# taohan10200/CRA5

Measured on AMD Instinct MI355X. Metric: ERA5 frames/s (721x1440x268) encode+decode, higher is better.
Workload: dtype f32 (3xf16-split MFMA, fp32 accumulate)

## Files before the change

cra5_amd/csrc/attention_split_f16.hip:

```cpp
#include <hip/hip_runtime.h>
#include <math.h>
#include <stdlib.h>

#include "../../include/cra5_amd.h"
#include "split.h"

CRA5_RANGE_TU(attn)

typedef float f32x16 __attribute__((ext_vector_type(16)));
typedef _Float16 half8 __attribute__((ext_vector_type(8)));
typedef _Float16 half4 __attribute__((ext_vector_type(4)));
typedef __fp16 fp16x4 __attribute__((__vector_size__(4 * sizeof(__fp16))));
#if defined(__HIP_DEVICE_COMPILE__)
#define CRA5_TR_READ(P) \
  __builtin_bit_cast(half4, __builtin_amdgcn_ds_read_tr16_b64_v4f16((__attribute__((address_space(3))) fp16x4 *)(P)))
#else
#define CRA5_TR_READ(P) (*reinterpret_cast<const half4 *>(P))
#endif

namespace {

__device__ __forceinline__ int xcd_remap(int bid, int nb) {
  const int q = nb / 8, r = nb % 8;
  const int xcd = bid % 8, within = bid / 8;
  const int base = (xcd < r) ? xcd * (q + 1) : r * (q + 1) + (xcd - r) * q;
  return base + within;
}

struct WinGeom {
  int H, W, wh, ww, nwc;
};

__device__ __forceinline__ int token_of(const WinGeom &g, int wr, int wc, int t) {
  if (g.ww == g.W && g.wh == g.H) return t;
  const int r = t / g.ww, c = t - r * g.ww;
  const int gr = wr * g.wh + r, gc = wc * g.ww + c;
  return (gr < g.H && gc < g.W) ? gr * g.W + gc : -1;
}

#ifdef CRA5_ATTN_TRACE
__device__ unsigned long long g_attn_trace[6 * 8192];
#define CRA5_ATRACE(SLOT, VAL)                                                                          \
  if (threadIdx.x == 0 && atrace_idx < 8192) g_attn_trace[atrace_idx * 6 + (SLOT)] = (VAL);
#else
#define CRA5_ATRACE(SLOT, VAL)
#endif

constexpr int HD = 64;
constexpr int KS = 72;
constexpr int VS = 96;
constexpr int MAX_WIN_TOKENS = 1152;

struct BalArgs {
  int groups;
  int n_full;
  int n_wg_pass;
  int rem_tile0;
  int rem;
  int n_grp;
  int nkt;
  int maxp;
  float *ws;
};
__host__ __device__ __forceinline__ long bal_cut(long S, int G, int c) { return S * c / G; }
__host__ __device__ __forceinline__ int bal_piece_of(long S, int G, long s) {
  int c = (int)(s * G / S);
  if (c > G - 1) c = G - 1;
  while (c > 0 && bal_cut(S, G, c) > s) --c;
  while (c < G - 1 && bal_cut(S, G, c + 1) <= s) ++c;
  return c;
}
constexpr int WS_ROW = 68;

template <int NW, bool HI, bool GLOBAL, bool BAL = false, bool PLAIN = false>
__global__ __launch_bounds__(NW * 64, (NW >= 8 ? 1 : (NW == 4 ? 3 : 2))) void window_attention_split_kernel(
    const unsigned short *__restrict__ qkv, long ldq ,
    const unsigned short *__restrict__ pad_row, float *__restrict__ out, unsigned short *__restrict__ out_s,
    int Kp_out, int C, int heads, WinGeom g, int q_tiles , float scale, BalArgs bal) {
  static_assert(!BAL || GLOBAL, "the balanced schedule is for whole-grid launches");
  static_assert(!PLAIN || HI, "plain rows carry no lo plane");
  constexpr int NT = NW * 64;
  constexpr int PPR = PLAIN ? 8 : 16;
  constexpr int PIECES = 32 * PPR;
  constexpr int STG = (PIECES + NT - 1) / NT;

  constexpr int KPL = 32 * KS + 32;
  constexpr int VPL = 32 * VS;
  constexpr int KBUF = 2 * KPL, VBUF = 2 * VPL;
  __shared__ __attribute__((aligned(16))) unsigned short lds[2 * KBUF + 2 * VBUF];
  unsigned short *Ks = lds;
  unsigned short *Vt = lds + 2 * KBUF;
  constexpr int TAB = GLOBAL ? 1 : MAX_WIN_TOKENS;
  __shared__ long long tab[TAB];

  const int L = g.wh * g.ww;
  int head, win, n_seg = 1;
  int seg_tile0[2] = {0, 0}, seg_nact[2] = {NW, NW}, seg_j0[2] = {0, 0}, seg_j1[2] = {L / 32, L / 32}, seg_part[2] = {-1, -1};
  int seg_grp[2] = {0, 0};
  if (BAL) {
    const int pass = blockIdx.x / bal.n_wg_pass, w = blockIdx.x - pass * bal.n_wg_pass;
    int slot;
    if ((heads & 7) == 0 && (bal.n_wg_pass & 7) == 0) {
      const int xcd = w & 7, s_ = w >> 3;
      head = xcd * (heads >> 3) + s_ / bal.groups;
      slot = s_ % bal.groups;
    } else {
      head = w / bal.groups;
      slot = w % bal.groups;
    }
    win = 0;
    if (pass < bal.n_full) {
      seg_tile0[0] = (pass * bal.groups + slot) * NW;
    } else {
      const long S = (long)bal.n_grp * bal.nkt;
      const long s0 = bal_cut(S, bal.groups, slot), s1 = bal_cut(S, bal.groups, slot + 1);
      n_seg = 0;
      for (long s = s0; s < s1;) {
        const int gq = (int)(s / bal.nkt);
        const long e = min(s1, (long)(gq + 1) * bal.nkt);
        if (n_seg < 2) {
          seg_grp[n_seg] = gq;
          seg_tile0[n_seg] = bal.rem_tile0 + gq * NW;
          seg_nact[n_seg] = min(NW, bal.rem - gq * NW);
          seg_j0[n_seg] = (int)(s - (long)gq * bal.nkt);
          seg_j1[n_seg] = (int)(e - (long)gq * bal.nkt);
          seg_part[n_seg] = slot - bal_piece_of(S, bal.groups, (long)gq * bal.nkt);
          ++n_seg;
        }
        s = e;
      }
    }
  } else {
    const int pid = xcd_remap(blockIdx.x, gridDim.x);
    const int qt = pid % q_tiles;
    const int wh_id = pid / q_tiles;
    head = wh_id % heads;
    win = wh_id / heads;
    seg_tile0[0] = qt * NW;
  }
  const int wr = win / g.nwc, wc = win - wr * g.nwc;

  const int tid = threadIdx.x, lane = tid & 63, wave = tid >> 6;
  const int l31 = lane & 31, h = lane >> 5;
  const int hoff = head * HD;
  const long qoff = (PLAIN ? 1L : 2L) * hoff, koff = (PLAIN ? 1L : 2L) * (C + hoff), voff = (PLAIN ? 1L : 2L) * (2 * C + hoff);

  if (!GLOBAL) {
    const long long pad_delta = reinterpret_cast<const char *>(pad_row) - reinterpret_cast<const char *>(qkv);
    for (int t = tid; t < L; t += NT) {
      const int tok = token_of(g, wr, wc, t);
      tab[t] = (tok >= 0) ? (long long)tok * ldq * 2 : pad_delta;
    }
  }
  constexpr bool IDLE_SKIP = !GLOBAL || BAL;
  bool tab_ready = GLOBAL;
#pragma unroll 1
  for (int seg = 0; seg < n_seg; ++seg) {
  const int tile0 = seg_tile0[seg], n_active = seg_nact[seg], j0 = seg_j0[seg], j1 = seg_j1[seg];
#ifdef CRA5_ATTN_TRACE
  const int atrace_idx = GLOBAL ? 8192 : (int)blockIdx.x;
  const unsigned long long atrace_c0 = clock64();
#endif
  CRA5_ATRACE(0, wall_clock64());
  const int tq = (tile0 + wave) * 32 + l31;
  const int q_tok = (tq < L && wave < n_active) ? token_of(g, wr, wc, tq) : -1;
  const bool wave_active = __any(q_tok >= 0);
  if (!__syncthreads_or(wave_active ? 1 : 0)) continue;
  tab_ready = true;

  half8 qh[4], ql[4];
  {
    const unsigned short *qrow = ((q_tok >= 0) ? qkv + (size_t)q_tok * ldq : pad_row) + qoff;
#pragma unroll
    for (int s = 0; s < 4; ++s) {
      const int chunk = s >> 1, pp = 2 * (s & 1) + h;
      if (PLAIN) {
        qh[s] = *reinterpret_cast<const half8 *>(qrow + 16 * s + 8 * h);
        ql[s] = qh[s];
      } else {
        qh[s] = *reinterpret_cast<const half8 *>(qrow + chunk * 64 + pp * 8);
        ql[s] = *reinterpret_cast<const half8 *>(qrow + chunk * 64 + 32 + pp * 8);
      }
    }
  }
  const float cexp = scale * 1.44269504088896340736f;
  f32x16 negm;
#pragma unroll
  for (int r = 0; r < 16; ++r) negm[r] = 0.f;
  if (HI) {
#pragma unroll
    for (int s = 0; s < 4; ++s)
#pragma unroll
      for (int e = 0; e < 8; ++e) qh[s][e] = (_Float16)((float)qh[s][e] * cexp);
  }
  const float cmax = HI ? 1.0f : cexp;

  f32x16 o[2];
#pragma unroll
  for (int t = 0; t < 2; ++t)
#pragma unroll
    for (int r = 0; r < 16; ++r) o[t][r] = 0.f;
  float m_run = HI ? 0.f : -INFINITY, l_run = 0.f;

  const int n_tiles = j1 - j0;
  uint4 sk0 = make_uint4(0u, 0u, 0u, 0u), sk1 = sk0, sv0 = sk0, sv1 = sk0;
  static_assert(STG == 1 || STG == 2, "staging below is written out for one or two 16-byte pieces per thread");
  constexpr bool TWO = STG == 2;
  const int krow0 = min(tid / PPR, 31), krow1 = min((tid + NT) / PPR, 31);
  const long kcol = koff + (tid % PPR) * 8;
  const long vcol = voff + (tid % PPR) * 8;
  const unsigned short *kq0 = qkv + (size_t)(krow0 + 32 * j0) * ldq + kcol;
  const unsigned short *kq1 = qkv + (size_t)(krow1 + 32 * j0) * ldq + kcol;
  const unsigned short *vq0 = qkv + (size_t)(krow0 + 32 * j0) * ldq + vcol;
  const unsigned short *vq1 = qkv + (size_t)(krow1 + 32 * j0) * ldq + vcol;
  const long tile_step = 32 * ldq;
#define CRA5_ROW(JJ, ROW) \
  reinterpret_cast<const unsigned short *>(reinterpret_cast<const char *>(qkv) + tab[(JJ)*32 + (ROW)])
  const bool stage0 = (NT <= PIECES) || (tid < PIECES);
  const bool stage1 = TWO && (tid + NT < PIECES);
#define CRA5_K_LOAD(J)                                                                    \
  if (stage0) {                                                                           \
    if (GLOBAL) {                                                                         \
      sk0 = *reinterpret_cast<const uint4 *>(kq0);                                        \
      if (stage1) sk1 = *reinterpret_cast<const uint4 *>(kq1);                            \
      const long st_ = ((J) < n_tiles - 1) ? tile_step : 0;  \
      kq0 += st_;                                                                         \
      kq1 += st_;                                                                         \
    } else {                                                                              \
      const int jj_ = min((J), n_tiles - 1);                                              \
      sk0 = *reinterpret_cast<const uint4 *>(CRA5_ROW(jj_, krow0) + kcol);                \
      if (stage1) sk1 = *reinterpret_cast<const uint4 *>(CRA5_ROW(jj_, krow1) + kcol);    \
    }                                                                                     \
  }
#define CRA5_V_LOAD(J)                                                                    \
  if (stage0) {                                                                           \
    if (GLOBAL) {                                                                         \
      sv0 = *reinterpret_cast<const uint4 *>(vq0);                                        \
      if (stage1) sv1 = *reinterpret_cast<const uint4 *>(vq1);                            \
      const long st_ = ((J) < n_tiles - 1) ? tile_step : 0;                               \
      vq0 += st_;                                                                         \
      vq1 += st_;                                                                         \
    } else {                                                                              \
      const int jj_ = min((J), n_tiles - 1);                                              \
      sv0 = *reinterpret_cast<const uint4 *>(CRA5_ROW(jj_, krow0) + vcol);                \
      if (stage1) sv1 = *reinterpret_cast<const uint4 *>(CRA5_ROW(jj_, krow1) + vcol);    \
    }                                                                                     \
  }
#define CRA5_K_STORE1(P, BUF)                                                             \
  {                                                                                       \
    const int idx = tid + (P)*NT;                                                         \
    if (idx < PIECES) {                                                                   \
      const int row = idx / PPR, piece = idx % PPR;                                       \
      const int plane = PLAIN ? 0 : (piece >> 2) & 1, d0 = PLAIN ? 8 * piece : 32 * (piece >> 3) + 8 * (piece & 3); \
      *reinterpret_cast<uint4 *>(Ks + (BUF)*KBUF + plane * KPL + row * KS + d0) = sk##P;  \
    }                                                                                     \
  }
#define CRA5_K_STORE(BUF) { CRA5_K_STORE1(0, BUF) if (TWO) CRA5_K_STORE1(1, BUF) }
#define CRA5_V_STORE1(P, BUF)                                                             \
  {                                                                                       \
    const int idx = tid + (P)*NT;                                                         \
    if (idx < PIECES) {                                                                   \
      const int row = idx / PPR, piece = idx % PPR;                                       \
      const int plane = PLAIN ? 0 : (piece >> 2) & 1, d0 = PLAIN ? 8 * piece : 32 * (piece >> 3) + 8 * (piece & 3); \
      *reinterpret_cast<uint4 *>(Vt + (BUF)*VBUF + plane * VPL + row * VS + d0) = sv##P;  \
    }                                                                                     \
  }
#define CRA5_V_STORE(BUF) { CRA5_V_STORE1(0, BUF) if (TWO) CRA5_V_STORE1(1, BUF) }
#define CRA5_SCORES(DST, KB)                                                              \
  {                                                                                       \
    f32x16 acc_;                                                                          \
    _Pragma("unroll") for (int r = 0; r < 16; ++r) acc_[r] = 0.f;                         \
    _Pragma("unroll") for (int st = 0; st < 4; ++st) {                                    \
      const half8 kh = *reinterpret_cast<const half8 *>(k_base + (KB)*KBUF + 16 * st);     \
      const half8 kl = *reinterpret_cast<const half8 *>(k_base + (KB)*KBUF + KPL + 16 * st); \
      if (!HI) {                                                                          \
        acc_ = __builtin_amdgcn_mfma_f32_32x32x16_f16(kl, qh[st], acc_, 0, 0, 0);         \
        acc_ = __builtin_amdgcn_mfma_f32_32x32x16_f16(kh, ql[st], acc_, 0, 0, 0);         \
      }                                                                                   \
      if (HI && st == 0) {                                                                \
        CRA5_MFMA_FROM(acc_, kh, qh[0], negm);                                            \
      } else {                                                                            \
        acc_ = __builtin_amdgcn_mfma_f32_32x32x16_f16(kh, qh[st], acc_, 0, 0, 0);         \
      }                                                                                   \
    }                                                                                     \
    DST = acc_;                                                                           \
  }
#if defined(__HIP_DEVICE_COMPILE__)
#define CRA5_MFMA_FROM(D, A, B, C) \
  asm("s_nop 3\n\tv_mfma_f32_32x32x16_f16 %0, %1, %2, %3" : "=&v"(D) : "v"(A), "v"(B), "v"(C))
#else
#define CRA5_MFMA_FROM(D, A, B, C) (D) = (C)
#endif

  const unsigned short *k_base = Ks + l31 * KS + 8 * h;
  const unsigned short *v_base = Vt + (4 * h + ((lane & 15) >> 2)) * VS + 16 * ((lane >> 4) & 1) + 4 * (lane & 3);

#if defined(__HIP_DEVICE_COMPILE__)
#define CRA5_XHALF_MAX(X)                                                                 \
  ({                                                                                      \
    float a_ = (X), b_ = (X), r_;                                                         \
    asm("s_nop 1\n\tv_permlane32_swap_b32_e32 %0, %1\n\ts_nop 1\n\tv_max_f32_e32 %2, %0, %1" \
        : "+v"(a_), "+v"(b_), "=v"(r_));                                                  \
    r_;                                                                                   \
  })
#define CRA5_MAX2_VALU(A, B)                                                              \
  ({                                                                                      \
    float r_;                                                                             \
    asm("v_max_f32_e32 %0, %1, %2" : "=v"(r_) : "v"(A), "v"(B));                          \
    r_;                                                                                   \
  })
#else
#define CRA5_XHALF_MAX(X) (X)
#define CRA5_MAX2_VALU(A, B) fmaxf((A), (B))
#endif
#if !defined(__HIP_DEVICE_COMPILE__)
#define CRA5_TILE_MAX(S)                                                                  \
  ({                                                                                      \
    float m_ = fmaxf(fmaxf(fmaxf(S[0], S[1]), fmaxf(S[2], S[3])), fmaxf(fmaxf(S[4], S[5]), fmaxf(S[6], S[7]))); \
    float n_ = fmaxf(fmaxf(fmaxf(S[8], S[9]), fmaxf(S[10], S[11])), fmaxf(fmaxf(S[12], S[13]), fmaxf(S[14], S[15]))); \
    CRA5_XHALF_MAX(fmaxf(m_, n_)) * cmax;       \
  })
#else
#define CRA5_MAX3(A, B, C) fmaxf(fmaxf((A), (B)), (C))
#define CRA5_TILE_MAX(S)                                                                  \
  ({                                                                                      \
    const float a_ = CRA5_MAX3(S[0], S[1], S[2]), b_ = CRA5_MAX3(S[3], S[4], S[5]), c_ = CRA5_MAX3(S[6], S[7], S[8]); \
    const float d_ = CRA5_MAX3(S[9], S[10], S[11]), e_ = CRA5_MAX3(S[12], S[13], S[14]);     \
    const float f_ = CRA5_MAX3(a_, b_, c_), g_ = CRA5_MAX3(d_, e_, S[15]);                   \
    CRA5_XHALF_MAX(CRA5_MAX2_VALU(f_, g_)) * cmax;  \
  })
#endif

  f32x16 s_cur;
  CRA5_K_LOAD(0);
  CRA5_V_LOAD(0);
  CRA5_K_STORE(0);
  CRA5_V_STORE(0);
  CRA5_K_LOAD(1);
  CRA5_K_STORE(1);
  __syncthreads();
  CRA5_K_LOAD(2);
  CRA5_V_LOAD(1);
  CRA5_SCORES(s_cur, 0);
  float mloc = CRA5_TILE_MAX(s_cur);
  __syncthreads();

  auto key_tile = [&](const int j, f32x16 &s_cur, f32x16 &s_next) __attribute__((always_inline)) {
    const int kb = (j + 1) & 1, vb = j & 1;
    if (!IDLE_SKIP || wave_active) {
    constexpr float DEFER_LOG2 = 8.0f;
    auto shift = [&](float delta, const bool rescale, f32x16 *also) __attribute__((always_inline)) {
      delta = (float)(_Float16)fminf(fmaxf(delta, -60000.f), 60000.f);
      if (rescale) {
        const float alpha = __builtin_amdgcn_exp2f(-delta);
        l_run *= alpha;
#pragma unroll
        for (int t = 0; t < 2; ++t)
#pragma unroll
          for (int r = 0; r < 16; ++r) o[t][r] *= alpha;
      }
      m_run += delta;
      half8 e0, bd;
#pragma unroll
      for (int e = 0; e < 8; ++e) {
        e0[e] = (_Float16)0.0f;
        bd[e] = (_Float16)0.0f;
      }
      e0[0] = (_Float16)(h == 0 ? 1.0f : 0.0f);
      bd[0] = (_Float16)(h == 0 ? -delta : 0.0f);
      s_cur = __builtin_amdgcn_mfma_f32_32x32x16_f16(e0, bd, s_cur, 0, 0, 0);
      negm = __builtin_amdgcn_mfma_f32_32x32x16_f16(e0, bd, negm, 0, 0, 0);
      if (also) *also = __builtin_amdgcn_mfma_f32_32x32x16_f16(e0, bd, *also, 0, 0, 0);
#if defined(__HIP_DEVICE_COMPILE__)
      asm volatile("s_nop 15\n\ts_nop 3" ::: "memory");
#endif
    };
    if (HI) {
      if (j == 0) shift(mloc, false, nullptr);
    } else if (!__all(mloc - m_run <= DEFER_LOG2)) {
      const float m_new = fmaxf(m_run, mloc);
      const float alpha = __builtin_amdgcn_exp2f(m_run - m_new);
      l_run *= alpha;
#pragma unroll
      for (int t = 0; t < 2; ++t)
#pragma unroll
        for (int r = 0; r < 16; ++r) o[t][r] *= alpha;
      m_run = m_new;
    }
    const float m_new = m_run;
#if defined(__HIP_DEVICE_COMPILE__)
    if (!HI) {
#define CRA5_FENCE() __builtin_amdgcn_sched_barrier(0)
#define CRA5_STAGE(MFMA_STMT) \
  CRA5_FENCE();               \
  MFMA_STMT;                  \
  CRA5_FENCE();
#define CRA5_KFRAG(PLANE, ST) (*reinterpret_cast<const half8 *>(k_base + kb * KBUF + (PLANE)*KPL + 16 * (ST)))
#define CRA5_MM(A, B, C) __builtin_amdgcn_mfma_f32_32x32x16_f16((A), (B), (C), 0, 0, 0)
      typedef _Float16 half2v __attribute__((ext_vector_type(2)));
      typedef unsigned u32x4 __attribute__((ext_vector_type(4)));
      float p[16], psum = 0.f;
      u32x4 phw[2], plw[2];
      auto exp_half = [&](const int u) __attribute__((always_inline)) {
        p[2 * u] = __builtin_amdgcn_exp2f(fmaf(s_cur[2 * u], cexp, -m_new));
        p[2 * u + 1] = __builtin_amdgcn_exp2f(fmaf(s_cur[2 * u + 1], cexp, -m_new));
      };
      auto split_half = [&](const int u) __attribute__((always_inline)) {
        const int r = 2 * u;
        const half2v h2 = {(_Float16)p[r], (_Float16)p[r + 1]};
        const unsigned hh = __builtin_bit_cast(unsigned, h2);
        float d0, d1;
        asm("v_fma_mix_f32 %0, %2, -1.0, %3 op_sel_hi:[1,0,0]\n\t"
            "v_fma_mix_f32 %1, %2, -1.0, %4 op_sel:[1,0,0] op_sel_hi:[1,0,0]"
            : "=&v"(d0), "=&v"(d1) : "v"(hh), "v"(p[r]), "v"(p[r + 1]));
        psum += p[r];
        psum += p[r + 1];
        const half2v l2 = {(_Float16)d0, (_Float16)d1};
        unsigned ll = __builtin_bit_cast(unsigned, l2);
        asm("" : "+v"(ll));
        phw[u >> 2][u & 3] = hh;
        plw[u >> 2][u & 3] = ll;
      };
#define ph(T) __builtin_bit_cast(half8, phw[T])
#define pl(T) __builtin_bit_cast(half8, plw[T])
      half8 vh[2], vl[2];
      auto v_frag = [&](const int t, const int plane, const int dt) __attribute__((always_inline)) {
        const unsigned short *vp = v_base + vb * VBUF + plane * VPL + 16 * t * VS + 32 * dt;
        const half4 a0 = CRA5_TR_READ(vp);
        const half4 a1 = CRA5_TR_READ(vp + 8 * VS);
        return __builtin_shufflevector(a0, a1, 0, 1, 2, 3, 4, 5, 6, 7);
      };
      half8 kh0 = CRA5_KFRAG(0, 0), kl0 = CRA5_KFRAG(1, 0), kh1 = CRA5_KFRAG(0, 1), kl1 = CRA5_KFRAG(1, 1);
      f32x16 acc;
#pragma unroll
      for (int r = 0; r < 16; ++r) acc[r] = 0.f;
      CRA5_STAGE(acc = CRA5_MM(kl0, qh[0], acc))
      exp_half(0);
      CRA5_STAGE(acc = CRA5_MM(kh0, ql[0], acc))
      exp_half(1);
      CRA5_STAGE(acc = CRA5_MM(kh0, qh[0], acc))
      split_half(0);
      const half8 kh2 = CRA5_KFRAG(0, 2), kl2 = CRA5_KFRAG(1, 2);
      CRA5_STAGE(acc = CRA5_MM(kl1, qh[1], acc))
      exp_half(2);
      CRA5_STAGE(acc = CRA5_MM(kh1, ql[1], acc))
      split_half(1);
      CRA5_STAGE(acc = CRA5_MM(kh1, qh[1], acc))
      exp_half(3);
      const half8 kh3 = CRA5_KFRAG(0, 3), kl3 = CRA5_KFRAG(1, 3);
      CRA5_STAGE(acc = CRA5_MM(kl2, qh[2], acc))
      split_half(2);
      CRA5_STAGE(acc = CRA5_MM(kh2, ql[2], acc))
      exp_half(4);
      CRA5_STAGE(acc = CRA5_MM(kh2, qh[2], acc))
      split_half(3);
      CRA5_STAGE(acc = CRA5_MM(kl3, qh[3], acc))
      exp_half(5);
      vl[0] = v_frag(0, 1, 0);
      vl[1] = v_frag(0, 1, 1);
      CRA5_STAGE(acc = CRA5_MM(kh3, ql[3], acc))
      split_half(4);
      CRA5_STAGE(acc = CRA5_MM(kh3, qh[3], acc))
      split_half(5);
      vh[0] = v_frag(0, 0, 0);
      vh[1] = v_frag(0, 0, 1);
      s_next = acc;
      CRA5_STAGE(o[0] = CRA5_MM(vl[0], ph(0), o[0]))
      exp_half(6);
      CRA5_STAGE(o[1] = CRA5_MM(vl[1], ph(0), o[1]))
      exp_half(7);
      CRA5_STAGE(o[0] = CRA5_MM(vh[0], pl(0), o[0]))
      split_half(6);
      CRA5_STAGE(o[1] = CRA5_MM(vh[1], pl(0), o[1]))
      split_half(7);
      vl[0] = v_frag(1, 1, 0);
      vl[1] = v_frag(1, 1, 1);
      CRA5_STAGE(o[0] = CRA5_MM(vh[0], ph(0), o[0]))
      l_run += psum;
      CRA5_STAGE(o[1] = CRA5_MM(vh[1], ph(0), o[1]))
      vh[0] = v_frag(1, 0, 0);
      vh[1] = v_frag(1, 0, 1);
      CRA5_STAGE(o[0] = CRA5_MM(vl[0], ph(1), o[0]))
      const float ma = CRA5_MAX3(s_next[0], s_next[1], s_next[2]), mb = CRA5_MAX3(s_next[3], s_next[4], s_next[5]);
      const float mc = CRA5_MAX3(s_next[6], s_next[7], s_next[8]), md = CRA5_MAX3(s_next[9], s_next[10], s_next[11]);
      const float me = CRA5_MAX3(s_next[12], s_next[13], s_next[14]);
      CRA5_STAGE(o[1] = CRA5_MM(vl[1], ph(1), o[1]))
      const float mf = CRA5_MAX3(ma, mb, mc), mg = CRA5_MAX3(md, me, s_next[15]);
      const float mfg = CRA5_MAX2_VALU(mf, mg);
      CRA5_STAGE(o[0] = CRA5_MM(vh[0], pl(1), o[0]))
      const float mx = CRA5_XHALF_MAX(mfg);
      CRA5_STAGE(o[1] = CRA5_MM(vh[1], pl(1), o[1]))
      mloc = mx * cmax;
      CRA5_STAGE(o[0] = CRA5_MM(vh[0], ph(1), o[0]))
      CRA5_STAGE(o[1] = CRA5_MM(vh[1], ph(1), o[1]))
#undef ph
#undef pl
#undef CRA5_MM
#undef CRA5_KFRAG
#undef CRA5_STAGE
#undef CRA5_FENCE
    } else
#endif
    {
    CRA5_SCORES(s_next, kb);
    float psum = 0.f;
    half8 ph[2], pl[2];
#if defined(__HIP_DEVICE_COMPILE__)
    if (HI) {
      typedef _Float16 half2v __attribute__((ext_vector_type(2)));
      typedef _Float16 half8v __attribute__((ext_vector_type(8)));
      const half2v ones = {(_Float16)1.0f, (_Float16)1.0f};
      auto exps = [&]() __attribute__((always_inline)) {
        psum = 0.f;
#pragma unroll
        for (int t = 0; t < 2; ++t) {
          half2v hp[4];
#pragma unroll
          for (int i = 0; i < 4; ++i) {
            hp[i] = half2v{(_Float16)__builtin_amdgcn_exp2f(s_cur[8 * t + 2 * i]), (_Float16)__builtin_amdgcn_exp2f(s_cur[8 * t + 2 * i + 1])};
            psum = __builtin_amdgcn_fdot2(hp[i], ones, psum, false);
          }
          ph[t] = half8v{hp[0][0], hp[0][1], hp[1][0], hp[1][1], hp[2][0], hp[2][1], hp[3][0], hp[3][1]};
        }
      };
      exps();
      constexpr float P_SAFE = 8192.0f;
      if (!__all(psum <= P_SAFE)) {
        const float mrel = CRA5_TILE_MAX(s_cur);
        shift(fmaxf(mrel, 0.f), true, &s_next);
        exps();
      }
#pragma unroll
      for (int t = 0; t < 2; ++t)
#pragma unroll
        for (int e = 0; e < 8; ++e) pl[t][e] = (_Float16)0.0f;
    }
#else
#pragma unroll
    for (int r = 0; r < 16; ++r) {
      const float p = HI ? (float)(_Float16)__builtin_amdgcn_exp2f(s_cur[r]) : __builtin_amdgcn_exp2f(fmaf(s_cur[r], cexp, -m_new));
      psum += p;
      const _Float16 hi = (_Float16)p;
      const _Float16 lo = (_Float16)(p - (float)hi);
      ph[r >> 3][r & 7] = hi;
      pl[r >> 3][r & 7] = lo;
    }
#endif
    l_run += psum;
#pragma unroll
    for (int t = 0; t < 2; ++t) {
      half8 vh[2], vl[2];
#pragma unroll
      for (int dt = 0; dt < 2; ++dt) {
        const unsigned short *vp = v_base + vb * VBUF + 16 * t * VS + 32 * dt;
        const unsigned short *vq = vp + VPL;
        const half4 a0 = CRA5_TR_READ(vp);
        const half4 a1 = CRA5_TR_READ(vp + 8 * VS);
        const half4 b0 = CRA5_TR_READ(vq);
        const half4 b1 = CRA5_TR_READ(vq + 8 * VS);
        vh[dt] = __builtin_shufflevector(a0, a1, 0, 1, 2, 3, 4, 5, 6, 7);
        vl[dt] = __builtin_shufflevector(b0, b1, 0, 1, 2, 3, 4, 5, 6, 7);
      }
      if (!HI) {
        o[0] = __builtin_amdgcn_mfma_f32_32x32x16_f16(vl[0], ph[t], o[0], 0, 0, 0);
        o[1] = __builtin_amdgcn_mfma_f32_32x32x16_f16(vl[1], ph[t], o[1], 0, 0, 0);
        o[0] = __builtin_amdgcn_mfma_f32_32x32x16_f16(vh[0], pl[t], o[0], 0, 0, 0);
        o[1] = __builtin_amdgcn_mfma_f32_32x32x16_f16(vh[1], pl[t], o[1], 0, 0, 0);
      }
      o[0] = __builtin_amdgcn_mfma_f32_32x32x16_f16(vh[0], ph[t], o[0], 0, 0, 0);
      o[1] = __builtin_amdgcn_mfma_f32_32x32x16_f16(vh[1], ph[t], o[1], 0, 0, 0);
    }
    if (!HI) mloc = CRA5_TILE_MAX(s_next);
    }
    }
    CRA5_K_STORE(j & 1);
    CRA5_V_STORE((j + 1) & 1);
    CRA5_K_LOAD(j + 3);
    CRA5_V_LOAD(j + 2);
    __syncthreads();
  };
  CRA5_ATRACE(1, wall_clock64());
  f32x16 s_alt;
  const int n_loop = n_tiles;
  int jt = 0;
  for (; jt + 1 < n_loop; jt += 2) {
    key_tile(jt, s_cur, s_alt);
    key_tile(jt + 1, s_alt, s_cur);
  }
  if (jt < n_loop) key_tile(jt, s_cur, s_alt);
  CRA5_ATRACE(2, wall_clock64());
  CRA5_ATRACE(4, (unsigned long long)n_tiles);

  const float l_tot = l_run + __shfl_xor(l_run, 32, 64);
  if (BAL && seg_part[seg] >= 0) {
    if (q_tok >= 0) {
      float *wrow = bal.ws + (((((size_t)head * bal.n_grp + seg_grp[seg]) * bal.maxp + seg_part[seg]) * NW + wave) * 32 + l31) * WS_ROW;
#pragma unroll
      for (int t = 0; t < 2; ++t)
#pragma unroll
        for (int gq = 0; gq < 4; ++gq) {
          const int d = 32 * t + 8 * gq + 4 * h;
          *reinterpret_cast<float4 *>(wrow + d) = make_float4(o[t][4 * gq + 0], o[t][4 * gq + 1], o[t][4 * gq + 2], o[t][4 * gq + 3]);
        }
      if (h == 0) {
        wrow[64] = m_run;
        wrow[65] = l_tot;
      }
    }
    continue;
  }
  {
    const bool live = q_tok >= 0;
    const float inv = live ? 1.0f / l_tot : 0.0f;
    float *orow = (out && live) ? out + (size_t)q_tok * C + hoff : nullptr;
    unsigned short *srow = (out_s && live) ? out_s + (size_t)q_tok * 2 * Kp_out : nullptr;
#pragma unroll
    for (int t = 0; t < 2; ++t)
#pragma unroll
      for (int pr = 0; pr < 2; ++pr) {
        float va[4], vb[4];
#pragma unroll
        for (int k = 0; k < 4; ++k) {
          va[k] = o[t][4 * (2 * pr) + k] * inv;
          vb[k] = o[t][4 * (2 * pr + 1) + k] * inv;
        }
        if (orow) {
          *reinterpret_cast<float4 *>(orow + 32 * t + 16 * pr + 4 * h) = make_float4(va[0], va[1], va[2], va[3]);
          *reinterpret_cast<float4 *>(orow + 32 * t + 16 * pr + 8 + 4 * h) = make_float4(vb[0], vb[1], vb[2], vb[3]);
        }
        if (out_s) {
          unsigned ha0, la0, ha1, la1, hb0, lb0, hb1, lb1;
          cra5_split_pair(va[0], va[1], ha0, la0);
          cra5_split_pair(va[2], va[3], ha1, la1);
          cra5_split_pair(vb[0], vb[1], hb0, lb0);
          cra5_split_pair(vb[2], vb[3], hb1, lb1);
#if defined(__HIP_DEVICE_COMPILE__)
#define CRA5_SWAP32(A, B)                                                  \
  {                                                                        \
    const auto r_ = __builtin_amdgcn_permlane32_swap((A), (B), false, false); \
    (A) = r_[0];                                                           \
    (B) = r_[1];                                                           \
  }
          CRA5_SWAP32(ha0, hb0);
          CRA5_SWAP32(ha1, hb1);
          CRA5_SWAP32(la0, lb0);
          CRA5_SWAP32(la1, lb1);
#undef CRA5_SWAP32
#endif
          if (srow) {
            const int c0 = hoff + 32 * t + 16 * pr + 8 * h;
            unsigned short *sp = srow + (PLAIN ? c0 : (c0 >> 5) * 64 + (c0 & 31));
            *reinterpret_cast<uint4 *>(sp) = make_uint4(ha0, ha1, hb0, hb1);
            if (!HI) *reinterpret_cast<uint4 *>(sp + 32) = make_uint4(la0, la1, lb0, lb1);
          }
        }
      }
  }
  CRA5_ATRACE(3, wall_clock64());
  CRA5_ATRACE(5, clock64() - atrace_c0);
  }
  (void)tab_ready;
}

__global__ __launch_bounds__(256) void attention_merge_kernel(const float *__restrict__ ws, float *__restrict__ out,
                                                              unsigned short *__restrict__ out_s, int Kp_out, int C,
                                                              BalArgs bal, int nw, int plain) {
  const int t = blockIdx.x % nw, hg = blockIdx.x / nw;
  const int grp = hg % bal.n_grp, head = hg / bal.n_grp;
  if (grp * nw + t >= bal.rem) return;
  const long S = (long)bal.n_grp * bal.nkt;
  const int c0 = bal_piece_of(S, bal.groups, (long)grp * bal.nkt);
  const int c1 = bal_piece_of(S, bal.groups, (long)(grp + 1) * bal.nkt - 1);
  const int np = c1 - c0 + 1;
  const int q = threadIdx.x >> 3, d0 = (threadIdx.x & 7) * 8;
  const size_t pstride = (size_t)nw * 32 * WS_ROW;
  const float *base = ws + ((((size_t)head * bal.n_grp + grp) * bal.maxp) * nw + t) * 32 * WS_ROW + (size_t)q * WS_ROW;
  float M = -INFINITY;
  for (int c = 0; c < np; ++c) M = fmaxf(M, base[c * pstride + 64]);
  float acc[8] = {0.f, 0.f, 0.f, 0.f, 0.f, 0.f, 0.f, 0.f}, lsum = 0.f;
  for (int c = 0; c < np; ++c) {
    const float *r = base + c * pstride;
    const float a = __builtin_amdgcn_exp2f(r[64] - M);
    lsum = fmaf(r[65], a, lsum);
    const float4 v0 = *reinterpret_cast<const float4 *>(r + d0), v1 = *reinterpret_cast<const float4 *>(r + d0 + 4);
    acc[0] = fmaf(v0.x, a, acc[0]);
    acc[1] = fmaf(v0.y, a, acc[1]);
    acc[2] = fmaf(v0.z, a, acc[2]);
    acc[3] = fmaf(v0.w, a, acc[3]);
    acc[4] = fmaf(v1.x, a, acc[4]);
    acc[5] = fmaf(v1.y, a, acc[5]);
    acc[6] = fmaf(v1.z, a, acc[6]);
    acc[7] = fmaf(v1.w, a, acc[7]);
  }
  const float inv = 1.0f / lsum;
  const int tok = (bal.rem_tile0 + grp * nw + t) * 32 + q, col = head * HD + d0;
#pragma unroll
  for (int k = 0; k < 8; ++k) acc[k] *= inv;
  if (out) {
    *reinterpret_cast<float4 *>(out + (size_t)tok * C + col) = make_float4(acc[0], acc[1], acc[2], acc[3]);
    *reinterpret_cast<float4 *>(out + (size_t)tok * C + col + 4) = make_float4(acc[4], acc[5], acc[6], acc[7]);
  }
  if (out_s) {
    unsigned short *srow = out_s + (size_t)tok * 2 * Kp_out;
    if (plain) {
      cra5_store_plain4(srow, col, acc[0], acc[1], acc[2], acc[3]);
      cra5_store_plain4(srow, col + 4, acc[4], acc[5], acc[6], acc[7]);
    } else {
      cra5_store_split4(srow, col, acc[0], acc[1], acc[2], acc[3]);
      cra5_store_split4(srow, col + 4, acc[4], acc[5], acc[6], acc[7]);
    }
  }
}

int cu_count() {
  static const int n = [] {
    int dev = 0, v = 0;
    if (hipGetDevice(&dev) != hipSuccess) return 256;
    if (hipDeviceGetAttribute(&v, hipDeviceAttributeMultiprocessorCount, dev) != hipSuccess || v <= 0) return 256;
    return v;
  }();
  return n;
}

constexpr int NW_GLOBAL = 12;

bool balanced_plan(int L, int heads, BalArgs &b) {
  const int P = cu_count(), T = L / 32;
  if (P % heads) return false;
  b.groups = P / heads;
  b.n_full = T / (b.groups * NW_GLOBAL);
  b.rem_tile0 = b.n_full * b.groups * NW_GLOBAL;
  b.rem = T - b.rem_tile0;
  b.n_grp = (b.rem + NW_GLOBAL - 1) / NW_GLOBAL;
  b.nkt = T;
  b.n_wg_pass = heads * b.groups;
  b.ws = nullptr;
  b.maxp = 0;
  const long S = (long)b.n_grp * b.nkt;
  for (int g = 0; g < b.n_grp; ++g) {
    const int np = bal_piece_of(S, b.groups, (long)(g + 1) * b.nkt - 1) - bal_piece_of(S, b.groups, (long)g * b.nkt) + 1;
    if (np > b.maxp) b.maxp = np;
  }
  if (!(b.n_full >= 1 && (b.rem == 0 || (b.n_grp <= b.groups && S >= b.groups)))) return false;
  for (int c = 0; b.rem && c < b.groups; ++c) {
    const long s0 = bal_cut(S, b.groups, c), s1 = bal_cut(S, b.groups, c + 1);
    if (s1 > s0 && (s1 - 1) / b.nkt - s0 / b.nkt + 1 > 2) return false;
  }
  return true;
}

size_t balanced_ws_bytes(const BalArgs &b, int heads) {
  return (size_t)heads * b.n_grp * b.maxp * NW_GLOBAL * 32 * WS_ROW * sizeof(float);
}

template <bool HI, bool PLAIN = false>
int launch_balanced(const unsigned short *qkv, long ldq, const unsigned short *pad_row, float *out, unsigned short *out_s,
                    int Kp_out, int C, int heads, int H, int W, float scale, BalArgs b, float *ws, hipStream_t st) {
  WinGeom g;
  g.H = H;
  g.W = W;
  g.wh = H;
  g.ww = W;
  g.nwc = 1;
  b.ws = ws;
  const int n_pass = b.n_full + (b.rem ? 1 : 0);
  hipLaunchKernelGGL((window_attention_split_kernel<NW_GLOBAL, HI, true, true, PLAIN>), dim3(n_pass * b.n_wg_pass),
                     dim3(NW_GLOBAL * 64), 0, st, qkv, ldq, pad_row, out, out_s, Kp_out, C, heads, g, 0, scale, b);
  int rc = (int)hipGetLastError();
  if (rc || b.rem == 0) return rc;
  hipLaunchKernelGGL(attention_merge_kernel, dim3(heads * b.n_grp * NW_GLOBAL), dim3(256), 0, st, ws, out, out_s, Kp_out,
                     C, b, NW_GLOBAL, PLAIN ? 1 : 0);
  return (int)hipGetLastError();
}

template <int NW, bool HI, bool GLOBAL, bool PLAIN = false>
int launch(const unsigned short *qkv, long ldq, const unsigned short *pad_row, float *out, unsigned short *out_s,
           int Kp_out, int C, int heads, int H, int W, int wh, int ww, float scale, hipStream_t st) {
  WinGeom g;
  g.H = H;
  g.W = W;
  g.wh = wh;
  g.ww = ww;
  const int nwr = (H + wh - 1) / wh;
  g.nwc = (W + ww - 1) / ww;
  const int L = wh * ww;
  const int q_tiles = (L + NW * 32 - 1) / (NW * 32);
  hipLaunchKernelGGL((window_attention_split_kernel<NW, HI, GLOBAL, false, PLAIN>), dim3(q_tiles * nwr * g.nwc * heads), dim3(NW * 64), 0, st,
                     qkv, ldq, pad_row, out, out_s, Kp_out, C, heads, g, q_tiles, scale, BalArgs{});
  return (int)hipGetLastError();
}

}

static int attention_dispatch(const uint16_t *qkv_split, int qkv_kp, const uint16_t *pad_row_split, float *out,
                              uint16_t *out_split, int out_kp, int C, int heads, int H, int W, int wh, int ww,
                              float scale, int hi_only, void *workspace, size_t workspace_bytes, void *stream,
                              bool want_balanced) {
  if (!qkv_split || !pad_row_split || (!out && !out_split) || heads <= 0 || C % heads) return CRA5_ERR_ARG;
  if (C / heads != 64 || qkv_kp != 3 * C) return CRA5_ERR_ARG;
  if (wh <= 0 || ww <= 0 || H <= 0 || W <= 0 || (wh * ww) % 32) return CRA5_ERR_ARG;
  if (out_split && (out_kp < C || out_kp % 32)) return CRA5_ERR_ARG;
  if (((uintptr_t)qkv_split & 15) || ((uintptr_t)pad_row_split & 15)) return CRA5_ERR_ARG;
  hipStream_t st = (hipStream_t)stream;
  const int L = wh * ww;
  if (hi_only != 0 && hi_only != 1 && hi_only != 3) return CRA5_ERR_ARG;
  const bool plain = hi_only == 3;
  const long ldq = 2L * qkv_kp;
  const bool whole = (wh == H && ww == W);
  if (!whole && L > MAX_WIN_TOKENS) return CRA5_ERR_ARG;
#define CRA5_ATT_GO(NWV, HIV, GLV) \
  return launch<NWV, HIV, GLV>(qkv_split, ldq, pad_row_split, out, out_split, out_kp, C, heads, H, W, wh, ww, scale, st)
  if (whole) {
    BalArgs b;
    if (want_balanced && balanced_plan(L, heads, b) &&
        (balanced_ws_bytes(b, heads) == 0 ||
         (workspace && ((uintptr_t)workspace & 15) == 0 && workspace_bytes >= balanced_ws_bytes(b, heads)))) {
      float *ws = reinterpret_cast<float *>(workspace);
      if (plain)
        return launch_balanced<true, true>(qkv_split, ldq, pad_row_split, out, out_split, out_kp, C, heads, H, W, scale, b, ws, st);
      if (hi_only)
        return launch_balanced<true>(qkv_split, ldq, pad_row_split, out, out_split, out_kp, C, heads, H, W, scale, b, ws, st);
      return launch_balanced<false>(qkv_split, ldq, pad_row_split, out, out_split, out_kp, C, heads, H, W, scale, b, ws, st);
    }
    if (plain) return launch<NW_GLOBAL, true, true, true>(qkv_split, ldq, pad_row_split, out, out_split, out_kp, C, heads, H, W, wh, ww, scale, st);
    if (hi_only) CRA5_ATT_GO(NW_GLOBAL, true, true);
    CRA5_ATT_GO(NW_GLOBAL, false, true);
  }
  if (plain) return launch<4, true, false, true>(qkv_split, ldq, pad_row_split, out, out_split, out_kp, C, heads, H, W, wh, ww, scale, st);
  if (hi_only) CRA5_ATT_GO(4, true, false);
  CRA5_ATT_GO(4, false, false);
#undef CRA5_ATT_GO
}

#ifdef CRA5_ATTN_TRACE
extern "C" int cra5_debug_attn_trace(unsigned long long *host, int n_rows) {
  if (n_rows < 1 || n_rows > 8192) return CRA5_ERR_ARG;
  if (hipDeviceSynchronize() != hipSuccess) return CRA5_ERR_ARG;
  int rc = (int)hipMemcpyFromSymbol(host, HIP_SYMBOL(g_attn_trace), sizeof(unsigned long long) * 6 * n_rows);
  void *p = nullptr;
  if (hipGetSymbolAddress(&p, HIP_SYMBOL(g_attn_trace)) == hipSuccess) hipMemset(p, 0, sizeof(unsigned long long) * 6 * 8192);
  return rc;
}
#endif

extern "C" int cra5_window_attention_split(const uint16_t *qkv_split, int qkv_kp, const uint16_t *pad_row_split,
                                           float *out, uint16_t *out_split, int out_kp, int C, int heads, int H,
                                           int W, int wh, int ww, float scale, int hi_only, void *stream) {
  return attention_dispatch(qkv_split, qkv_kp, pad_row_split, out, out_split, out_kp, C, heads, H, W, wh, ww, scale,
                            hi_only, nullptr, 0, stream, false);
}

extern "C" size_t cra5_attention_workspace_bytes(int n_tokens, int heads) {
  BalArgs b;
  if (n_tokens <= 0 || heads <= 0 || (n_tokens % 32) || !balanced_plan(n_tokens, heads, b)) return 0;
  return balanced_ws_bytes(b, heads);
}

extern "C" int cra5_window_attention_split_ws(const uint16_t *qkv_split, int qkv_kp, const uint16_t *pad_row_split,
                                              float *out, uint16_t *out_split, int out_kp, int C, int heads, int H,
                                              int W, int wh, int ww, float scale, int hi_only, void *workspace,
                                              size_t workspace_bytes, void *stream) {
  return attention_dispatch(qkv_split, qkv_kp, pad_row_split, out, out_split, out_kp, C, heads, H, W, wh, ww, scale,
                            hi_only, workspace, workspace_bytes, stream, true);
}

extern "C" int cra5_attention_balanced_plan(int n_tokens, int heads, size_t *workspace_bytes) {
  BalArgs b;
  if (workspace_bytes) *workspace_bytes = 0;
  if (n_tokens <= 0 || heads <= 0 || (n_tokens % 32) || !balanced_plan(n_tokens, heads, b)) return 0;
  if (workspace_bytes) *workspace_bytes = balanced_ws_bytes(b, heads);
  return 1;
}
```

Before: 31.68.

## Skip padded query groups in edge windows and collapse padded key tiles

Windowed attention launches now count only the query tiles that hold real tokens in each edge, bottom or corner window, so no workgroup is spent on all-padding query groups, and live tiles are spread evenly across the remaining waves. For the non-HI windowed path, padded key tiles, which all carry the same pad row, reuse one precomputed exp/split of the scores and a fixed V fragment. This avoids reloading K/V and recomputing scores for those tiles. The change adds more complex index decoding per block and a separate tail loop, and correctness depends on every padded key tile being identical.

```diff
diff --git a/cra5_amd/csrc/attention_split_f16.hip b/cra5_amd/csrc/attention_split_f16.hip
--- a/cra5_amd/csrc/attention_split_f16.hip
+++ b/cra5_amd/csrc/attention_split_f16.hip
@@ -37,6 +37,16 @@
   const int gr = wr * g.wh + r, gc = wc * g.ww + c;
   return (gr < g.H && gc < g.W) ? gr * g.W + gc : -1;
 }
+
+__host__ __device__ __forceinline__ int live_tiles(const WinGeom &g, int wr, int wc) {
+  const int lr = (g.H - wr * g.wh < g.wh) ? g.H - wr * g.wh : g.wh, lc = (g.W - wc * g.ww < g.ww) ? g.W - wc * g.ww : g.ww;
+  return ((lr - 1) * g.ww + lc + 31) / 32;
+}
+struct WinPack {
+  int n_in, n_right, n_bottom, n_corner;
+  int col_wgs;
+  int nwr;
+};
 
 #ifdef CRA5_ATTN_TRACE
 __device__ unsigned long long g_attn_trace[6 * 8192];
@@ -76,10 +86,11 @@
 __global__ __launch_bounds__(NW * 64, (NW >= 8 ? 1 : (NW == 4 ? 3 : 2))) void window_attention_split_kernel(
     const unsigned short *__restrict__ qkv, long ldq ,
     const unsigned short *__restrict__ pad_row, float *__restrict__ out, unsigned short *__restrict__ out_s,
-    int Kp_out, int C, int heads, WinGeom g, int q_tiles , float scale, BalArgs bal) {
+    int Kp_out, int C, int heads, WinGeom g, WinPack pk , float scale, BalArgs bal) {
   static_assert(!BAL || GLOBAL, "the balanced schedule is for whole-grid launches");
   static_assert(!PLAIN || HI, "plain rows carry no lo plane");
   constexpr int NT = NW * 64;
+  constexpr bool PAD_SKIP = !GLOBAL && !HI;
   constexpr int PPR = PLAIN ? 8 : 16;
   constexpr int PIECES = 32 * PPR;
   constexpr int STG = (PIECES + NT - 1) / NT;
@@ -94,7 +105,8 @@
   __shared__ long long tab[TAB];
 
   const int L = g.wh * g.ww;
-  int head, win, n_seg = 1;
+  int head, wr = 0, wc = 0, n_seg = 1;
+  int n_live = L / 32;
   int seg_tile0[2] = {0, 0}, seg_nact[2] = {NW, NW}, seg_j0[2] = {0, 0}, seg_j1[2] = {L / 32, L / 32}, seg_part[2] = {-1, -1};
   int seg_grp[2] = {0, 0};
   if (BAL) {
@@ -108,7 +120,6 @@
       head = w / bal.groups;
       slot = w % bal.groups;
     }
-    win = 0;
     if (pass < bal.n_full) {
       seg_tile0[0] = (pass * bal.groups + slot) * NW;
     } else {
@@ -132,13 +143,22 @@
     }
   } else {
     const int pid = xcd_remap(blockIdx.x, gridDim.x);
-    const int qt = pid % q_tiles;
-    const int wh_id = pid / q_tiles;
-    head = wh_id % heads;
-    win = wh_id / heads;
-    seg_tile0[0] = qt * NW;
-  }
-  const int wr = win / g.nwc, wc = win - wr * g.nwc;
+    wc = min(pid / pk.col_wgs, g.nwc - 1);
+    int rem = pid - wc * pk.col_wgs;
+    const bool right = wc == g.nwc - 1;
+    const int n_a = right ? pk.n_right : pk.n_in, n_b = right ? pk.n_corner : pk.n_bottom;
+    const int per_head = (pk.nwr - 1) * n_a + n_b;
+    head = rem / per_head;
+    rem -= head * per_head;
+    wr = min(rem / n_a, pk.nwr - 1);
+    const int grp = rem - wr * n_a;
+    const int ng = (wr == pk.nwr - 1) ? n_b : n_a;
+    n_live = live_tiles(g, wr, wc);
+    const bool even = !GLOBAL && n_live < L / 32;
+    const int per = even ? n_live / ng : NW, extra = even ? n_live - per * ng : 0;
+    seg_tile0[0] = grp * per + min(grp, extra);
+    seg_nact[0] = even ? per + (grp < extra ? 1 : 0) : min(NW, n_live - grp * NW);
+  }
 
   const int tid = threadIdx.x, lane = tid & 63, wave = tid >> 6;
   const int l31 = lane & 31, h = lane >> 5;
@@ -345,10 +365,55 @@
   float mloc = CRA5_TILE_MAX(s_cur);
   __syncthreads();
 
+  constexpr float DEFER_LOG2 = 8.0f;
+  auto raise_max = [&]() __attribute__((always_inline)) {
+    if (!__all(mloc - m_run <= DEFER_LOG2)) {
+      const float m_new = fmaxf(m_run, mloc);
+      const float alpha = __builtin_amdgcn_exp2f(m_run - m_new);
+      l_run *= alpha;
+#pragma unroll
+      for (int t = 0; t < 2; ++t)
+#pragma unroll
+        for (int r = 0; r < 16; ++r) o[t][r] *= alpha;
+      m_run = m_new;
+      return true;
+    }
+    return false;
+  };
+#if defined(__HIP_DEVICE_COMPILE__)
+  typedef _Float16 half2v __attribute__((ext_vector_type(2)));
+  typedef unsigned u32x4 __attribute__((ext_vector_type(4)));
+  auto exp_unit = [&](float *p, const f32x16 &s, const float m_ref, const int u) __attribute__((always_inline)) {
+    p[2 * u] = __builtin_amdgcn_exp2f(fmaf(s[2 * u], cexp, -m_ref));
+    p[2 * u + 1] = __builtin_amdgcn_exp2f(fmaf(s[2 * u + 1], cexp, -m_ref));
+  };
+  auto split_unit = [&](const float *p, float &psum, u32x4 *phw, u32x4 *plw, const int u) __attribute__((always_inline)) {
+    const int r = 2 * u;
+    const half2v h2 = {(_Float16)p[r], (_Float16)p[r + 1]};
+    const unsigned hh = __builtin_bit_cast(unsigned, h2);
+    float d0, d1;
+    asm("v_fma_mix_f32 %0, %2, -1.0, %3 op_sel_hi:[1,0,0]\n\t"
+        "v_fma_mix_f32 %1, %2, -1.0, %4 op_sel:[1,0,0] op_sel_hi:[1,0,0]"
+        : "=&v"(d0), "=&v"(d1) : "v"(hh), "v"(p[r]), "v"(p[r + 1]));
+    psum += p[r];
+    psum += p[r + 1];
+    const half2v l2 = {(_Float16)d0, (_Float16)d1};
+    unsigned ll = __builtin_bit_cast(unsigned, l2);
+    asm("" : "+v"(ll));
+    phw[u >> 2][u & 3] = hh;
+    plw[u >> 2][u & 3] = ll;
+  };
+  auto v_frag_at = [&](const int vb, const int t, const int plane, const int dt) __attribute__((always_inline)) {
+    const unsigned short *vp = v_base + vb * VBUF + plane * VPL + 16 * t * VS + 32 * dt;
+    const half4 a0 = CRA5_TR_READ(vp);
+    const half4 a1 = CRA5_TR_READ(vp + 8 * VS);
+    return __builtin_shufflevector(a0, a1, 0, 1, 2, 3, 4, 5, 6, 7);
+  };
+#endif
+
   auto key_tile = [&](const int j, f32x16 &s_cur, f32x16 &s_next) __attribute__((always_inline)) {
     const int kb = (j + 1) & 1, vb = j & 1;
     if (!IDLE_SKIP || wave_active) {
-    constexpr float DEFER_LOG2 = 8.0f;
     auto shift = [&](float delta, const bool rescale, f32x16 *also) __attribute__((always_inline)) {
       delta = (float)(_Float16)fminf(fmaxf(delta, -60000.f), 60000.f);
       if (rescale) {
@@ -377,15 +442,8 @@
     };
     if (HI) {
       if (j == 0) shift(mloc, false, nullptr);
-    } else if (!__all(mloc - m_run <= DEFER_LOG2)) {
-      const float m_new = fmaxf(m_run, mloc);
-      const float alpha = __builtin_amdgcn_exp2f(m_run - m_new);
-      l_run *= alpha;
-#pragma unroll
-      for (int t = 0; t < 2; ++t)
-#pragma unroll
-        for (int r = 0; r < 16; ++r) o[t][r] *= alpha;
-      m_run = m_new;
+    } else {
+      raise_max();
     }
     const float m_new = m_run;
 #if defined(__HIP_DEVICE_COMPILE__)
@@ -397,38 +455,15 @@
   CRA5_FENCE();
 #define CRA5_KFRAG(PLANE, ST) (*reinterpret_cast<const half8 *>(k_base + kb * KBUF + (PLANE)*KPL + 16 * (ST)))
 #define CRA5_MM(A, B, C) __builtin_amdgcn_mfma_f32_32x32x16_f16((A), (B), (C), 0, 0, 0)
-      typedef _Float16 half2v __attribute__((ext_vector_type(2)));
-      typedef unsigned u32x4 __attribute__((ext_vector_type(4)));
       float p[16], psum = 0.f;
       u32x4 phw[2], plw[2];
-      auto exp_half = [&](const int u) __attribute__((always_inline)) {
-        p[2 * u] = __builtin_amdgcn_exp2f(fmaf(s_cur[2 * u], cexp, -m_new));
-        p[2 * u + 1] = __builtin_amdgcn_exp2f(fmaf(s_cur[2 * u + 1], cexp, -m_new));
-      };
-      auto split_half = [&](const int u) __attribute__((always_inline)) {
-        const int r = 2 * u;
-        const half2v h2 = {(_Float16)p[r], (_Float16)p[r + 1]};
-        const unsigned hh = __builtin_bit_cast(unsigned, h2);
-        float d0, d1;
-        asm("v_fma_mix_f32 %0, %2, -1.0, %3 op_sel_hi:[1,0,0]\n\t"
-            "v_fma_mix_f32 %1, %2, -1.0, %4 op_sel:[1,0,0] op_sel_hi:[1,0,0]"
-            : "=&v"(d0), "=&v"(d1) : "v"(hh), "v"(p[r]), "v"(p[r + 1]));
-        psum += p[r];
-        psum += p[r + 1];
-        const half2v l2 = {(_Float16)d0, (_Float16)d1};
-        unsigned ll = __builtin_bit_cast(unsigned, l2);
-        asm("" : "+v"(ll));
-        phw[u >> 2][u & 3] = hh;
-        plw[u >> 2][u & 3] = ll;
-      };
+      auto exp_half = [&](const int u) __attribute__((always_inline)) { exp_unit(p, s_cur, m_new, u); };
+      auto split_half = [&](const int u) __attribute__((always_inline)) { split_unit(p, psum, phw, plw, u); };
 #define ph(T) __builtin_bit_cast(half8, phw[T])
 #define pl(T) __builtin_bit_cast(half8, plw[T])
       half8 vh[2], vl[2];
       auto v_frag = [&](const int t, const int plane, const int dt) __attribute__((always_inline)) {
-        const unsigned short *vp = v_base + vb * VBUF + plane * VPL + 16 * t * VS + 32 * dt;
-        const half4 a0 = CRA5_TR_READ(vp);
-        const half4 a1 = CRA5_TR_READ(vp + 8 * VS);
-        return __builtin_shufflevector(a0, a1, 0, 1, 2, 3, 4, 5, 6, 7);
+        return v_frag_at(vb, t, plane, dt);
       };
       half8 kh0 = CRA5_KFRAG(0, 0), kl0 = CRA5_KFRAG(1, 0), kh1 = CRA5_KFRAG(0, 1), kl1 = CRA5_KFRAG(1, 1);
       f32x16 acc;
@@ -581,13 +616,57 @@
   };
   CRA5_ATRACE(1, wall_clock64());
   f32x16 s_alt;
-  const int n_loop = n_tiles;
+  const bool pad_tail = PAD_SKIP && n_live < n_tiles;
+  const int n_loop = pad_tail ? n_live : n_tiles;
   int jt = 0;
   for (; jt + 1 < n_loop; jt += 2) {
     key_tile(jt, s_cur, s_alt);
     key_tile(jt + 1, s_alt, s_cur);
   }
-  if (jt < n_loop) key_tile(jt, s_cur, s_alt);
+  if (jt < n_loop) {
+    key_tile(jt, s_cur, s_alt);
+    if (pad_tail) s_cur = s_alt;
+  }
+#if defined(__HIP_DEVICE_COMPILE__)
+  if (PAD_SKIP && pad_tail && wave_active) {
+    const int vb = n_loop & 1;
+    float p[16], psum = 0.f;
+    u32x4 phw[2], plw[2];
+    half8 vh[2][2], vl[2][2];
+#pragma unroll
+    for (int t = 0; t < 2; ++t)
+#pragma unroll
+      for (int dt = 0; dt < 2; ++dt) {
+        vl[t][dt] = v_frag_at(vb, t, 1, dt);
+        vh[t][dt] = v_frag_at(vb, t, 0, dt);
+      }
+    bool p_valid = false;
+#pragma unroll 1
+    for (int j = n_loop; j < n_tiles; ++j) {
+      if (raise_max()) p_valid = false;
+      if (!p_valid) {
+        psum = 0.f;
+#pragma unroll
+        for (int u = 0; u < 8; ++u) exp_unit(p, s_cur, m_run, u);
+        __builtin_amdgcn_sched_barrier(0);
+#pragma unroll
+        for (int u = 0; u < 8; ++u) split_unit(p, psum, phw, plw, u);
+        p_valid = true;
+      }
+      l_run += psum;
+#pragma unroll
+      for (int t = 0; t < 2; ++t) {
+        const half8 ph = __builtin_bit_cast(half8, phw[t]), pl = __builtin_bit_cast(half8, plw[t]);
+        o[0] = __builtin_amdgcn_mfma_f32_32x32x16_f16(vl[t][0], ph, o[0], 0, 0, 0);
+        o[1] = __builtin_amdgcn_mfma_f32_32x32x16_f16(vl[t][1], ph, o[1], 0, 0, 0);
+        o[0] = __builtin_amdgcn_mfma_f32_32x32x16_f16(vh[t][0], pl, o[0], 0, 0, 0);
+        o[1] = __builtin_amdgcn_mfma_f32_32x32x16_f16(vh[t][1], pl, o[1], 0, 0, 0);
+        o[0] = __builtin_amdgcn_mfma_f32_32x32x16_f16(vh[t][0], ph, o[0], 0, 0, 0);
+        o[1] = __builtin_amdgcn_mfma_f32_32x32x16_f16(vh[t][1], ph, o[1], 0, 0, 0);
+      }
+    }
+  }
+#endif
   CRA5_ATRACE(2, wall_clock64());
   CRA5_ATRACE(4, (unsigned long long)n_tiles);
 
@@ -765,7 +844,7 @@
   b.ws = ws;
   const int n_pass = b.n_full + (b.rem ? 1 : 0);
   hipLaunchKernelGGL((window_attention_split_kernel<NW_GLOBAL, HI, true, true, PLAIN>), dim3(n_pass * b.n_wg_pass),
-                     dim3(NW_GLOBAL * 64), 0, st, qkv, ldq, pad_row, out, out_s, Kp_out, C, heads, g, 0, scale, b);
+                     dim3(NW_GLOBAL * 64), 0, st, qkv, ldq, pad_row, out, out_s, Kp_out, C, heads, g, WinPack{}, scale, b);
   int rc = (int)hipGetLastError();
   if (rc || b.rem == 0) return rc;
   hipLaunchKernelGGL(attention_merge_kernel, dim3(heads * b.n_grp * NW_GLOBAL), dim3(256), 0, st, ws, out, out_s, Kp_out,
@@ -783,10 +862,17 @@
   g.ww = ww;
   const int nwr = (H + wh - 1) / wh;
   g.nwc = (W + ww - 1) / ww;
-  const int L = wh * ww;
-  const int q_tiles = (L + NW * 32 - 1) / (NW * 32);
-  hipLaunchKernelGGL((window_attention_split_kernel<NW, HI, GLOBAL, false, PLAIN>), dim3(q_tiles * nwr * g.nwc * heads), dim3(NW * 64), 0, st,
-                     qkv, ldq, pad_row, out, out_s, Kp_out, C, heads, g, q_tiles, scale, BalArgs{});
+  auto groups = [&](int wr, int wc) { return (live_tiles(g, wr, wc) + NW - 1) / NW; };
+  WinPack pk;
+  pk.nwr = nwr;
+  pk.n_in = groups(0, 0);
+  pk.n_right = groups(0, g.nwc - 1);
+  pk.n_bottom = groups(nwr - 1, 0);
+  pk.n_corner = groups(nwr - 1, g.nwc - 1);
+  pk.col_wgs = heads * ((nwr - 1) * pk.n_in + pk.n_bottom);
+  const int n_wgs = (g.nwc - 1) * pk.col_wgs + heads * ((nwr - 1) * pk.n_right + pk.n_corner);
+  hipLaunchKernelGGL((window_attention_split_kernel<NW, HI, GLOBAL, false, PLAIN>), dim3(n_wgs), dim3(NW * 64), 0, st,
+                     qkv, ldq, pad_row, out, out_s, Kp_out, C, heads, g, pk, scale, BalArgs{});
   return (int)hipGetLastError();
 }
 
```

After: 31.65. Within noise of the previous version (-0.1%).
